# wmeddie/CycloneML

Hardware: AMD Instinct MI355X
Metric: rows/s per training iteration (higher is better)
Workload: dtype f64

## Files before the change

### cycloneml_amd/csrc/kmeans.hip

```cpp
#pragma clang fp contract(off)

#include <hip/hip_runtime.h>

#include <algorithm>
#include <cmath>
#include <cstdlib>
#include <mutex>
#include <utility>
#include <vector>

#include "common.hpp"
#include "kmeans_centers.hpp"
#include "kmeans_i8.hpp"
#include "kmeans_cos.hpp"
#include "kmeans_fp64.hpp"
#include "kmeans_sparse.hpp"
#include "kmeans_sums.hpp"
#include "silhouette.hpp"

namespace {

using cyc::kmsums::kChunkRows;
using cyc::kmsums::kMaxK;

bool env_is0(const char* name) {
  const char* e = std::getenv(name);
  return e && e[0] == '0';
}
int sw_assign_variant() {
  const char* v = std::getenv("CYC_KMEANS_ASSIGN");
  return v ? std::atoi(v) : 0;
}
bool sw_cands3() { return !env_is0("CYC_KMEANS_CANDS3"); }
bool sw_refine() { return std::getenv("CYC_KMEANS_NO_REFINE") == nullptr; }
bool sw_stage() { return std::getenv("CYC_KMEANS_NO_STAGE") == nullptr; }
bool sw_bounds() {
  static const bool on = !env_is0("CYC_KMEANS_BOUNDS");
  return on;
}
bool sw_nbr() {
  static const bool on = !env_is0("CYC_KMEANS_NBR");
  return on;
}
bool sw_incr() {
  static const bool on = !env_is0("CYC_KMEANS_INCR");
  return on;
}
bool sw_exact_split() {
  static const bool on = !env_is0("CYC_KMEANS_EXACT_SPLIT");
  return on;
}
bool sw_list16() {
  static const bool on = !env_is0("CYC_KMEANS_LIST_BM");
  return on;
}
int sw_dump_call() {
  static const int call = [] {
    const char* e = std::getenv("CYC_KMEANS_DUMP_CALL");
    return e ? std::atoi(e) : 10;
  }();
  return call;
}

constexpr int kNormRows = 256, kNormCols = 16, kNormStride = kNormCols + 1;
__global__ __launch_bounds__(kNormRows) void k_row_norms(const double* __restrict__ X, int64_t n,
                                                         int d, double* __restrict__ norms) {
  __shared__ double tile[2][kNormRows * kNormStride];
  const int t = threadIdx.x;
  const int64_t row0 = (int64_t)blockIdx.x * kNormRows;
  constexpr int PER = kNormRows * kNormCols / kNormRows;
  double v[PER];
  auto load = [&](int c0) {
#pragma unroll
    for (int i = 0; i < PER; ++i) {
      const int e = t + kNormRows * i, r = e / kNormCols, c = c0 + e % kNormCols;
      const int64_t gr = row0 + r;
      v[i] = (gr < n && c < d) ? __builtin_nontemporal_load(&X[gr * d + c]) : 0.0;
    }
  };
  auto store = [&](double* b) {
#pragma unroll
    for (int i = 0; i < PER; ++i) {
      const int e = t + kNormRows * i;
      b[(e / kNormCols) * kNormStride + e % kNormCols] = v[i];
    }
  };
// ... 104 lines not shown
    if (c0 + kNormCols < d) store(tile[buf ^ 1]);
    buf ^= 1;
  }
  if (myr < n) cost[myr] = s;
}

}

struct cyc_kmeans_plan_s {
  int d = 0, k = 0;
  int measure = CYC_DISTANCE_EUCLIDEAN;
  cyc::DeviceBuffer cosV, cosVn, cosCn;
  bool dense_ok = true;
  cyc::kmfp64::Sizing fp;
  int64_t lastTier2 = 0;
  int64_t lastExact = 0;
  int64_t lastLimb3 = -1;
  int64_t lastCands = -1;
  int64_t lastCands2 = -1;
  bool cands3 = false;
  cyc::DeviceBuffer cb3, cq3, ok3, list3, list3Count;
  int ktp8 = 0;
  cyc::DeviceBuffer cb8, cq8, g8, prm8, scr8, list8Count;
  cyc::DeviceBuffer candRows, cands, candCount;
  cyc::DeviceBuffer candRows2, cands2, candCount2;
  cyc::DeviceBuffer cand1Rows, cand1, cand1Count, fullList, fullCount;
  cyc::DeviceBuffer stgRowsA, stgRowsB, stgCandRows, stgCands, stgCounts;
  bool lastRefined = false;
  int64_t max_rows = 0;
  std::mutex mu;
  cyc::DeviceBuffer ct, stats, dmin, slowList, slowCount, assignTmp, costTmp;
  cyc::kmsums::SortScratch sort;
  cyc::DeviceBuffer exactDist;
  cyc::DeviceBuffer req;
  cyc::DeviceBuffer silFlags, silNorms, silPart;
  unsigned long long* reqHost = nullptr;
  hipEvent_t reqEv = nullptr;
  ~cyc_kmeans_plan_s() {
    if (reqHost) (void)hipHostFree(reqHost);
    if (reqEv) (void)hipEventDestroy(reqEv);
  }
};

struct cyc_kmeans_rows_s {
  const double* X = nullptr;
  int64_t n = 0;
  int d = 0;
  bool usable = false;
  bool cosine = false;
  cyc::DeviceBuffer img, meta, unorm;
  bool bEnabled = true;
  bool bValid = false;
  int bk = 0;
  cyc::DeviceBuffer bnd, bAssign, bCp, bDelta, bCcs, bPrm, bTmp, bCount, bList, bListCount, bCum;
  cyc::DeviceBuffer bTmp2, bCount2;
  cyc::DeviceBuffer bLnc, bSets, bState, bRc, bRcCount, bRcCum;
  cyc::DeviceBuffer bNbr, bNbrR;
  int64_t bCalls = 0, bFullRows = 0;
  cyc::kmsums::IncState inc;
};

namespace {

int do_stats(cyc_kmeans_plan p, const double* C, hipStream_t st) {
  const int k = p->k, d = p->d;
  const int tps = (k + kStT - 1) / kStT;
// ... 254 lines not shown
                       i8 ? (unsigned int*)p->list3Count.ptr : nullptr);
    CYC_LAUNCH_CHECK("k_zero2");
  }
  int rc = CYC_OK;
  const int32_t* rowList = nullptr;
  const unsigned int* rowCount = nullptr;
  if (i8) {
    if (!a.prepared &&
        (rc = cyc::km8::centers_prepare(C, cnorm, p->k, p->d, p->ktp8, p->cb8.ptr,
                                        (float*)p->cq8.ptr, (double*)p->g8.ptr,
                                        (cyc::km8::CenterParams*)p->prm8.ptr,
                                        (double*)p->scr8.ptr, st)))
      return rc;
    cyc::km8::ScreenCall sc = ss.call;
    sc.xnorm = xnorm;
    sc.assign = a.assign;
    sc.st = st;
    if ((rc = cyc::km8::screen(sc, (int32_t*)p->list3.ptr, (unsigned int*)p->list3Count.ptr,
                               slowList, (unsigned int*)p->list8Count.ptr, ss.cand(),
                               ss.refine(), ss.stage(), a.bounds, a.prepared)))
      return rc;
    rowList = (const int32_t*)p->list3.ptr;
    rowCount = (const unsigned int*)p->list3Count.ptr;
  } else if (fp.variant == 3) {
    if ((rc = cyc::kmfp64::launch_assign3(fp, X, xnorm, n, C, cnorm, p->cb3.ptr,
                                          (float*)p->cq3.ptr, (int*)p->ok3.ptr, a.assign, a.cost,
                                          (int32_t*)p->list3.ptr,
                                          (unsigned int*)p->list3Count.ptr, st)))
      return rc;
    rowList = (const int32_t*)p->list3.ptr;
    rowCount = (const unsigned int*)p->list3Count.ptr;
  }
  const int bm = rowList && sw_list16() && fp.bm >= 16 ? 16 : fp.bm;
  if ((rc = cyc::kmfp64::launch_assign(fp, bm, X, xnorm, n, C, cnorm, ct, a.assign, a.cost,
                                       slowList, slowCount, st, rowList, rowCount)))
    return rc;
  int64_t known = -1;
  if (a.n_exact_out) {
    unsigned int h_slow = 0, h_tier2 = 0, h_limb3 = 0, h_cand = 0, h_cand2 = 0;
    const bool twoPass = i8 && cyc::km8::uses32(p->d);
    CYC_HIP(hipMemcpyAsync(&h_slow, slowCount, sizeof(unsigned), hipMemcpyDeviceToHost, st));
    if (rowCount)
      CYC_HIP(hipMemcpyAsync(&h_tier2, rowCount, sizeof(unsigned), hipMemcpyDeviceToHost, st));
    if (twoPass) {
      CYC_HIP(hipMemcpyAsync(&h_limb3, p->list8Count.ptr, sizeof(unsigned), hipMemcpyDeviceToHost, st));
      CYC_HIP(hipMemcpyAsync(&h_cand, p->candCount.ptr, sizeof(unsigned), hipMemcpyDeviceToHost, st));
      if (p->cands3)
        CYC_HIP(hipMemcpyAsync(&h_cand2, p->candCount2.ptr, sizeof(unsigned), hipMemcpyDeviceToHost, st));
    }
    CYC_HIP(hipStreamSynchronize(st));
    *a.n_exact_out = h_slow;
    p->lastTier2 = rowCount ? (int64_t)h_tier2 : n;
    p->lastExact = h_slow;
    p->lastLimb3 = twoPass ? (int64_t)h_limb3 : -1;
    p->lastCands = twoPass ? (int64_t)h_cand : -1;
    p->lastCands2 = twoPass && p->cands3 ? (int64_t)h_cand2 : -1;
    if (!h_slow) return CYC_OK;
    known = h_slow;
  }
  return cyc::kmfp64::launch_exact(fp, X, xnorm, n, C, cnorm, ct, statsArg, slowList, slowCount,
                                   p->exactDist, a.assign, a.cost, a.approxNorm, known,
                                   sw_exact_split(), st);
}

int req_reserve(cyc_kmeans_plan p, size_t bytes) {
  int rc;
  if ((rc = p->req.reserve(bytes))) return rc;
  if (!p->reqHost) CYC_HIP(hipHostMalloc((void**)&p->reqHost, 5 * sizeof(unsigned long long)));
  if (!p->reqEv) CYC_HIP(hipEventCreateWithFlags(&p->reqEv, hipEventDisableTiming));
  return CYC_OK;
}

int require_enqueue(cyc_kmeans_plan p, const double* C, const double* xnorm, int64_t n,
                    hipStream_t st) {
  int rc;
  if ((rc = req_reserve(p, 5 * sizeof(unsigned long long)))) return rc;
  CYC_HIP(hipMemsetAsync(p->req.ptr, 0xff, 2 * sizeof(unsigned long long), st));
  const int64_t work = std::max<int64_t>(n, (int64_t)p->k * p->d);
  const unsigned grid = (unsigned)std::max<int64_t>(1, std::min<int64_t>((work + 255) / 256, 2048));
  hipLaunchKernelGGL(k_require_norms, dim3(grid), dim3(256), 0, st, C, p->k, p->d, xnorm, n,
                     (unsigned long long*)p->req.ptr);
  CYC_LAUNCH_CHECK("k_require_norms");
  CYC_HIP(hipMemcpyAsync(p->reqHost, p->req.ptr, 5 * sizeof(unsigned long long),
                         hipMemcpyDeviceToHost, st));
  CYC_HIP(hipEventRecord(p->reqEv, st));
  return CYC_OK;
}

int prep_all(cyc_kmeans_plan p, cyc_kmeans_rows rows, const double* xnorm, int64_t n,
             const double* C, const double* cnorm, bool useBnd, bool carry,
             const ScreenSetup* ss, hipStream_t st) {
  namespace k8 = cyc::km8;
  const int k = p->k, d = p->d;
  int rc;
  const size_t reqBytes = sizeof(unsigned long long) * (8 + (size_t)k);
// ... 203 lines not shown
  auto* p = new cyc_kmeans_plan_s();
  p->d = d;
  p->k = k;
  p->fp = cyc::kmfp64::sizing(d, k, sw_assign_variant());
  p->dense_ok = p->fp.bm != 0;
  int rc;
  if (p->fp.variant == 3 &&
      ((rc = p->cb3.reserve((size_t)p->fp.ktp3 * p->fp.ks3 * 2 * 64 * 16)) ||
       (rc = p->cq3.reserve(sizeof(float) * (size_t)p->fp.ktp3 * 16)) ||
       (rc = p->ok3.reserve(64)))) {
    delete p;
    return rc;
  }
  if ((rc = p->list3Count.reserve(64))) {
    delete p;
    return rc;
  }
  if (d <= cyc::km8::kMaxD) {
    const int ks8 = cyc::km8::ksteps(d);
    p->ktp8 = (int)cyc::round_up((k + 15) / 16, cyc::km8::kWaves);
    if ((rc = p->cb8.reserve((size_t)p->ktp8 * ks8 * 3 * 64 * 16 * 2)) ||
        (rc = p->cq8.reserve(sizeof(float) * (size_t)p->ktp8 * 48)) ||
        (rc = p->g8.reserve(sizeof(double) * (size_t)p->ktp8 * 48)) ||
        (rc = p->list8Count.reserve(64)) ||
        (rc = p->prm8.reserve(sizeof(cyc::km8::CenterParams))) ||
        (rc = p->scr8.reserve(sizeof(double) * 2 * (size_t)k))) {
      delete p;
      return rc;
    }
  }
  if ((p->dense_ok && (rc = p->ct.reserve(sizeof(double) * (size_t)p->fp.d4 * p->fp.kpad))) ||
      (rc = p->stats.reserve(sizeof(double) * ((size_t)k * (k + 1) / 2))) ||
      (rc = p->dmin.reserve(sizeof(unsigned long long) * (size_t)k)) ||
      (rc = p->slowCount.reserve(64)) || (rc = ensure_rows(p, std::max<int64_t>(max_rows, 1)))) {
    delete p;
    return rc;
  }
  *plan = p;
  return CYC_OK;
}

int cyc_kmeans_last_tiers(cyc_kmeans_plan p, int64_t* fp64_screen_rows, int64_t* exact_rows) {
  CYC_REQUIRE(p != nullptr && fp64_screen_rows && exact_rows, "arguments must not be null");
  std::lock_guard<std::mutex> g(p->mu);
  *fp64_screen_rows = p->lastTier2;
  *exact_rows = p->lastExact;
  return CYC_OK;
}

int cyc_kmeans_last_screen(cyc_kmeans_plan p, int64_t* three_limb_rows) {
  CYC_REQUIRE(p != nullptr && three_limb_rows, "arguments must not be null");
  std::lock_guard<std::mutex> g(p->mu);
  *three_limb_rows = p->lastLimb3;
  return CYC_OK;
}

int cyc_kmeans_last_candidates(cyc_kmeans_plan p, int64_t* candidate_rows) {
  CYC_REQUIRE(p != nullptr && candidate_rows, "arguments must not be null");
  std::lock_guard<std::mutex> g(p->mu);
  *candidate_rows = p->lastCands;
  return CYC_OK;
}

int cyc_kmeans_last_candidates3(cyc_kmeans_plan p, int64_t* fp64_rows) {
  CYC_REQUIRE(p != nullptr && fp64_rows, "arguments must not be null");
  std::lock_guard<std::mutex> g(p->mu);
  *fp64_rows = p->lastCands2;
// ... 590 lines not shown
```

### cycloneml_amd/csrc/kmeans_fp64.hip

```cpp
#pragma clang fp contract(off)

#include <hip/hip_runtime.h>

#include <algorithm>

#include "common.hpp"
#include "kmeans_fp64.hpp"

namespace {

constexpr int kWaves = 8;
constexpr int kAssignThreads = kWaves * 64;

struct Slot {
  float L1, U1, L2;
  int I1;
};

__device__ __forceinline__ float ulp_down(float f) {
  int b = __float_as_int(f);
  if (f == 0.0f) return -__int_as_float(1);
  return __int_as_float(f > 0.0f ? b - 1 : b + 1);
}
__device__ __forceinline__ float f_down(double x) {
// ... 186 lines not shown
  }
  __syncthreads();

  if (tid < rows) {
    const int row = tid;
    Slot S{__builtin_inff(), __builtin_inff(), __builtin_inff(), -1};
    for (int w = 0; w < kWaves; ++w) {
      const double* m = mrg + ((size_t)w * BM + row) * 4;
      slot_merge(S, (float)m[0], (float)m[1], (float)m[2], (int)m[3]);
    }
    const int64_t grow = CYC_GROW1(row);
    if (S.I1 >= 0 && S.L2 > S.U1) {
      if (cost) {
        const double* crow = C + (int64_t)S.I1 * d;
        const double* xrow = Xs + row * ldsStride;
        double s = 0.0;
        for (int j = 0; j < d; ++j) {
          double sc = dsub(crow[j], xrow[j]);
          s = dadd(s, dmul(sc, sc));
        }
        cost[grow] = s;
      }
      assign[grow] = S.I1;
    } else {
      unsigned slot = atomicAdd(slowCount, 1u);
      slowList[slot] = (int32_t)grow;
    }
  }
  __syncthreads();
  }
#undef CYC_GROW1
}

template <int BM>
__global__ __launch_bounds__(kAssignThreads, 1) void k_kmeans_assign2(
    const double* __restrict__ X, const double* __restrict__ xnorm, int64_t n, int d, int d4,
    int ldsStride, const double* __restrict__ Ct, const double* __restrict__ C,
    const double* __restrict__ cnorm, int k, int kpad, double marginFac,
    int32_t* __restrict__ assign, double* __restrict__ cost, int32_t* __restrict__ slowList,
    unsigned int* __restrict__ slowCount, const int32_t* __restrict__ rowList,
    const unsigned int* __restrict__ rowCount) {
  constexpr int T = BM / 16;
  extern __shared__ __attribute__((aligned(16))) double smem[];
  double* Xs = smem;
  double* xnS = Xs + BM * ldsStride;
  double* mrg = xnS + BM;
  double* cnS = mrg + kWaves * BM * 4;
  double* xqS = cnS + kpad;
  const int64_t nsrc = rowList ? (int64_t)*rowCount : n;
  for (int64_t blk = blockIdx.x; blk * BM < nsrc; blk += gridDim.x) {
#define CYC_GROW(i) (rowList ? (int64_t)rowList[row0 + (i)] : row0 + (i))
  const double fac2 = 2.0 * marginFac;

  const int tid = threadIdx.x, lane = tid & 63;
  const int wave = __builtin_amdgcn_readfirstlane(tid >> 6);
  const int64_t row0 = blk * BM;
  const int rows = (int)min<int64_t>(BM, nsrc - row0);
  {
    const int total = rows * d;
    for (int e = tid; e < total; e += kAssignThreads) {
      int r = e / d, c = e - r * d;
      Xs[r * ldsStride + c] = X[CYC_GROW(r) * d + c];
    }
    for (int e = tid; e < BM * d4; e += kAssignThreads) {
      int r = e / d4, c = e - r * d4;
      if (r >= rows || c >= d) Xs[r * ldsStride + c] = 0.0;
    }
    if (tid < BM) {
      const double xn = (tid < rows) ? xnorm[CYC_GROW(tid)] : 0.0;
      xnS[tid] = xn;
      xqS[tid] = (xn * xn) * (1.0 - fac2);
    }
    for (int c = tid; c < kpad; c += kAssignThreads) cnS[c] = c < k ? cnorm[c] : 0.0;
  }
  __syncthreads();
  const auto ctR = __builtin_amdgcn_make_buffer_rsrc((void*)Ct, (short)0, d4 * kpad * 8,
                                                     0x00020000);
  const int laneOff = ((lane >> 4) * kpad + (lane & 15)) * 8;

  float sL1[T * 4], sL2[T * 4];
  int sI1[T * 4];
#pragma unroll
  for (int q = 0; q < T * 4; ++q) {
    sL1[q] = sL2[q] = __builtin_inff();
    sI1[q] = -1;
  }
  unsigned poison = 0;
  const double* arow = Xs + (lane & 15) * ldsStride + (lane >> 4);
  cyc_double4 acc[T];
  const int G = d4 / 32;
  const int nslabs = (kpad - wave * 16 + kWaves * 16 - 1) / (kWaves * 16);
  const int total = nslabs * G;
  double b0[8], b1[8];

#define CYC_LOADB(B, I)                                                              \
  do {                                                                               \
    const int nb_ = wave * 16 + ((I) / G) * (kWaves * 16);                           \
    const int so_ = ((((I) % G) * 32) * kpad + nb_) * 8;                             \
    _Pragma("unroll") for (int s = 0; s < 8; ++s)                                    \
      B[s] = __builtin_bit_cast(double, __builtin_amdgcn_raw_buffer_load_b64(          \
          ctR, laneOff, so_ + s * 32 * kpad, 0));                                    \
  } while (0)
#define CYC_COMPUTE(B, I)                                                            \
  do {                                                                               \
    const int g_ = (I) % G;                                                          \
    if (g_ == 0) {                                                                   \
      _Pragma("unroll") for (int t = 0; t < T; ++t) acc[t] = cyc_double4{0.0, 0.0, 0.0, 0.0}; \
    }                                                                                \
    _Pragma("unroll") for (int s = 0; s < 8; ++s) {                                  \
      _Pragma("unroll") for (int t = 0; t < T; ++t) {                                \
        const double a_ = arow[t * 16 * ldsStride + g_ * 32 + s * 4];                \
        acc[t] = __builtin_amdgcn_mfma_f64_16x16x4f64(a_, B[s], acc[t], 0, 0, 0);    \
      }                                                                              \
    }                                                                                \
    if (g_ == G - 1) {                                                               \
      const int c_ = wave * 16 + ((I) / G) * (kWaves * 16) + (lane & 15);            \
      const double cn_ = cnS[c_];                                                    \
      const double cq_ = (cn_ * cn_) * (1.0 - fac2);                                 \
      const bool cok_ = c_ < k;                                                      \
      _Pragma("unroll") for (int t = 0; t < T; ++t) {                                \
        _Pragma("unroll") for (int r = 0; r < 4; ++r) {                              \
          const int q = 4 * t + r;                                                   \
          const double xq = xqS[t * 16 + (lane >> 4) + 4 * r];                       \
          const double L = (xq + cq_) - (acc[t][r] + acc[t][r]);                      \
          poison |= (cok_ && !(L == L)) ? (1u << q) : 0u;                            \
          const float fL = (float)L;      \
          const bool lt = cok_ && fL < sL1[q];                                       \
          const float l2 = cok_ ? fminf(sL2[q], fL) : sL2[q];                        \
          sL2[q] = lt ? sL1[q] : l2;                                                 \
          sI1[q] = lt ? c_ : sI1[q];                                                 \
          sL1[q] = lt ? fL : sL1[q];                                                 \
        }                                                                            \
      }                                                                              \
    }                                                                                \
  } while (0)
  __builtin_amdgcn_s_setreg(0x801, 2);
  if (total > 0) CYC_LOADB(b0, 0);
  for (int i = 0; i < total; i += 2) {
    if (i + 1 < total) CYC_LOADB(b1, i + 1);
    CYC_COMPUTE(b0, i);
    if (i + 2 < total) CYC_LOADB(b0, i + 2);
    if (i + 1 < total) CYC_COMPUTE(b1, i + 1);
  }
  __builtin_amdgcn_s_setreg(0x801, 0);
#undef CYC_LOADB
#undef CYC_COMPUTE

#pragma unroll
  for (int q = 0; q < T * 4; ++q) {
#pragma unroll
    for (int m = 1; m < 16; m <<= 1) {
      const float oL1 = __shfl_xor(sL1[q], m), oL2 = __shfl_xor(sL2[q], m);
      const int oI1 = __shfl_xor(sI1[q], m);
      const float hi = fmaxf(sL1[q], oL1);
      sL2[q] = fminf(hi, fminf(sL2[q], oL2));
      const bool take = oL1 < sL1[q] || (oL1 == sL1[q] && oI1 >= 0 && (sI1[q] < 0 || oI1 < sI1[q]));
      sI1[q] = take ? oI1 : sI1[q];
      sL1[q] = take ? oL1 : sL1[q];
    }
  }
#pragma unroll
  for (int m = 1; m < 16; m <<= 1) poison |= __shfl_xor(poison, m);
  if ((lane & 15) == 0) {
#pragma unroll
    for (int t = 0; t < T; ++t) {
#pragma unroll
      for (int r = 0; r < 4; ++r) {
        const int q = 4 * t + r;
        double* m = mrg + ((size_t)wave * BM + t * 16 + (lane >> 4) + 4 * r) * 4;
        m[0] = sL1[q];
        m[1] = ((poison >> q) & 1u) ? -__builtin_inf() : (double)sL2[q];
        m[2] = (double)sI1[q];
      }
    }
  }
  __syncthreads();

  if (tid < rows) {
    const int row = tid;
    float L1 = __builtin_inff(), L2 = __builtin_inff();
    int I1 = -1;
    for (int w = 0; w < kWaves; ++w) {
      const double* m = mrg + ((size_t)w * BM + row) * 4;
      const float oL1 = (float)m[0], oL2 = (float)m[1];
      const int oI1 = (int)m[2];
      const float hi = fmaxf(L1, oL1);
      L2 = fminf(hi, fminf(L2, oL2));
      if (oL1 < L1 || (oL1 == L1 && oI1 >= 0 && (I1 < 0 || oI1 < I1))) {
        L1 = oL1;
        I1 = oI1;
      }
    }
    const int64_t grow = CYC_GROW(row);
    bool decided = false;
    if (I1 >= 0 && L1 == L1 && L1 < __builtin_inff()) {
      const double xn = xnS[row], cn = cnS[I1];
      const double M = (xn * xn + cn * cn) * fac2;
      const double U = (double)(-ulp_down(-L1)) + 2.0 * M * (1.0 + 0x1p-40);
      decided = (double)L2 > U;
    }
    if (decided) {
      if (cost) {
        const double* crow = C + (int64_t)I1 * d;
        const double* xrow = Xs + row * ldsStride;
        double s = 0.0;
        for (int j = 0; j < d; ++j) {
          double sc = dsub(crow[j], xrow[j]);
          s = dadd(s, dmul(sc, sc));
        }
        cost[grow] = s;
      }
      assign[grow] = I1;
    } else {
      unsigned slot = atomicAdd(slowCount, 1u);
      slowList[slot] = (int32_t)grow;
    }
  }
  __syncthreads();
  }
#undef CYC_GROW
}

typedef __bf16 cyc_bf16x8 __attribute__((ext_vector_type(8)));
typedef float cyc_float4 __attribute__((ext_vector_type(4)));

// ... 268 lines not shown
                                                    const int32_t* __restrict__ slowList,
                                                    const unsigned int* __restrict__ slowCount,
                                                    double* __restrict__ dist) {
  __shared__ double xs[1280];
  const unsigned cnt = *slowCount;
  const unsigned idx = blockIdx.y;
  if (cnt > (unsigned)kExactCap || idx >= cnt) return;
  const int tid = threadIdx.x;
  const int c = blockIdx.x * 256 + tid;
  const int64_t r = slowList[idx];
  const double* x = X + r * d;
  const bool xl = d <= 1280;
  if (xl)
    for (int j = tid; j < d; j += 256) xs[j] = x[j];
  __syncthreads();
  const double* xv = xl ? xs : x;
  double acc = 0.0;
  for (int j0 = 0; j0 < d; j0 += 16) {
    double cv[16];
#pragma unroll
    for (int jj = 0; jj < 16; ++jj)
      cv[jj] = (j0 + jj < d && c < k) ? Ct[(int64_t)(j0 + jj) * kpad + c] : 0.0;
#pragma unroll
    for (int jj = 0; jj < 16; ++jj) {
      if (j0 + jj < d) {
        const double sc = dsub(cv[jj], xv[j0 + jj]);
        acc = dadd(acc, dmul(sc, sc));
      }
    }
  }
  if (c < k) dist[(int64_t)idx * kpad + c] = acc;
}

__global__ __launch_bounds__(64) void k_exact_replay(const double* __restrict__ X,
                                                     const double* __restrict__ xnorm, int d,
                                                     int kpad, const double* __restrict__ cnorm,
                                                     int k, const double* __restrict__ stats,
                                                     const int32_t* __restrict__ slowList,
                                                     const unsigned int* __restrict__ slowCount,
                                                     const double* __restrict__ dist,
                                                     int32_t* __restrict__ assign,
                                                     double* __restrict__ cost, int exactNorm) {
  const unsigned cnt = *slowCount;
  const unsigned idx = blockIdx.x;
  if (cnt > (unsigned)kExactCap || idx >= cnt) return;
  const int lane = threadIdx.x;
  const int64_t r = slowList[idx];
  const bool ns = stats == nullptr;
  double xn = 0.0;
  if (exactNorm) {
    if (lane == 0) xn = seq_norm2(X + r * d, d);
    xn = __shfl(xn, 0);
  } else {
    xn = xnorm[r];
  }
  const double* dds = dist + (int64_t)idx * kpad;
  double best = __builtin_inf();
  int bi = 0;
  bool done = false;
  int first = 0;
  if (!ns) {
    best = dds[0];
    done = best < stats[0];
    first = 1;
  }
  for (int i0 = first; !done && i0 < k; i0 += 64) {
    const int i = i0 + lane;
    const bool valid = i < k;
    double lb = __builtin_inf(), sii = 0.0, dd = 0.0;
    if (valid) {
      const double nd = dsub(cnorm[i], xn);
      lb = dmul(nd, nd);
      sii = ns ? 0.0 : stats[iut(i, i)];
      dd = dds[i];
    }
    int pos = 0;
    for (;;) {
      const bool visit = valid && lane >= pos && lb < best && (ns || stats[iut(i, bi)] < best);
      const bool brk = !ns && visit && dd < sii;
      const bool ev = visit && (brk || dd < best);
      const unsigned long long m = __ballot(ev);
      if (!m) break;
      const int f = __ffsll((long long)m) - 1;
      best = __shfl(dd, f);
      bi = i0 + f;
      if (__shfl((int)brk, f)) {
        done = true;
        break;
      }
      pos = f + 1;
    }
  }
  if (lane == 0) {
    assign[r] = bi;
    if (cost) cost[r] = best;
  }
}

constexpr int kExactChunk = 1024;
constexpr int kExactX = 1280;

__global__ __launch_bounds__(256) void k_assign_exact(
    const double* __restrict__ X, const double* __restrict__ xnorm, int d,
    const double* __restrict__ C, const double* __restrict__ Ct, int kpad,
    const double* __restrict__ cnorm, int k,
    const double* __restrict__ stats, const int32_t* __restrict__ slowList,
    const unsigned int* __restrict__ slowCount, int32_t* __restrict__ assign,
    double* __restrict__ cost, int exactNorm, unsigned int skipUpTo) {
  __shared__ double xs[kExactX];
  __shared__ double dds[kExactChunk];
  __shared__ int doneS;
  __shared__ double xnS;
  const unsigned cnt = *slowCount;
  if (cnt <= skipUpTo) return;
  const int tid = threadIdx.x, lane = tid & 63;
  const bool ns = stats == nullptr;
  for (unsigned idx = blockIdx.x; idx < cnt; idx += gridDim.x) {
    const int64_t r = slowList[idx];
    const double* x = X + r * d;
    __syncthreads();
    const bool xl = d <= kExactX;
    if (xl)
      for (int j = tid; j < d; j += 256) xs[j] = x[j];
    const double* xv = xl ? xs : x;
    if (exactNorm) {
      __syncthreads();
      if (tid == 0) xnS = seq_norm2(xv, d);
      __syncthreads();
// ... 74 lines not shown
    }
    if (tid == 0) {
      assign[r] = bi;
      if (cost) cost[r] = best;
    }
  }
}

}

namespace cyc {
namespace kmfp64 {

namespace {

constexpr int kS3TB = 2;

int pick_bm(int d4, int& stride, size_t& lds) {
  const int cands[3] = {64, 32, 16};
  const int maxbm = 64;
  for (int bm : cands) {
    if (bm > maxbm) continue;
    int s = d4 + ((2 - d4 % 32) + 32) % 32;
    size_t bytes = ((size_t)bm * s + bm + (size_t)kWaves * bm * 4) * sizeof(double);
    if (bytes <= 160 * 1024) {
      stride = s;
      lds = bytes;
      return bm;
    }
  }
  return 0;
}

template <int BM>
int launch_assign_bm(const Sizing& s, const double* X, const double* xnorm, int64_t n,
                     const double* C, const double* cnorm, const double* ct, int32_t* assign,
                     double* cost, int32_t* slowList, unsigned int* slowCount, hipStream_t st,
                     const int32_t* rowList, const unsigned int* rowCount) {
  static bool attr_set = false;
  if (!attr_set) {
    CYC_HIP(hipFuncSetAttribute((const void*)k_kmeans_assign<BM>,
                                hipFuncAttributeMaxDynamicSharedMemorySize, 160 * 1024));
    CYC_HIP(hipFuncSetAttribute(reinterpret_cast<const void*>(&k_kmeans_assign2<BM>),
                                hipFuncAttributeMaxDynamicSharedMemorySize, 160 * 1024));
    attr_set = true;
  }
  const double marginFac = (double)(s.d + 16) * 0x1p-46;
  const int64_t blocks = rowList ? std::min<int64_t>((n + BM - 1) / BM, 1024) : (n + BM - 1) / BM;
  cyc::KernelTimer timer(rowList ? "k_kmeans_assign_fp64" : "k_kmeans_assign", st);
  if (s.variant == 2 || s.variant == 3)
    hipLaunchKernelGGL(HIP_KERNEL_NAME(k_kmeans_assign2<BM>), dim3((unsigned)blocks),
                       dim3(kAssignThreads), s.assignLds2, st, X, xnorm, n, s.d, s.d4,
                       s.ldsStride2, ct, C, cnorm, s.k, s.kpad, marginFac, assign, cost, slowList,
                       slowCount, rowList, rowCount);
  else
    hipLaunchKernelGGL(k_kmeans_assign<BM>, dim3((unsigned)blocks), dim3(kAssignThreads),
                       s.assignLds, st, X, xnorm, n, s.d, s.d4, s.ldsStride, ct, C, cnorm, s.k,
                       s.kpad, marginFac, assign, cost, slowList, slowCount, rowList, rowCount);
  CYC_LAUNCH_CHECK("k_kmeans_assign");
  return CYC_OK;
}

}

Sizing sizing(int d, int k, int want) {
  Sizing s;
  s.d = d;
  s.k = k;
  s.d4 = (int)cyc::round_up(d, 4);
  s.kpad = (int)cyc::round_up(k, 16);
  s.bm = pick_bm(s.d4, s.ldsStride, s.assignLds);
  s.ldsStride2 = s.d4 + 1;
  s.assignLds2 = s.assignLds + sizeof(double) * ((size_t)s.kpad + s.bm) -
                 sizeof(double) * (size_t)s.bm * (s.ldsStride - s.ldsStride2);
  s.variant = ((s.d4 % 32) == 0 && s.assignLds2 <= 160 * 1024) ? 2 : 1;
  s.ks3 = (int)((d + 31) / 32);
  s.lds3 = (size_t)2 * kS3BM * (s.ks3 * 4 + 1) * 16 + (size_t)kS3Waves * kS3BM * 12 +
           (size_t)kS3BM * 8;
  const bool fits3 = s.variant == 2 && s.lds3 <= 160 * 1024;
  if (fits3) s.variant = 3;
  if (want == 1 || (s.d4 % 32 == 0 && s.assignLds2 <= 160 * 1024 && want >= 2 && want <= 3 &&
                    (want != 3 || fits3)))
    s.variant = want;
  s.ktp3 = (int)cyc::round_up((k + 15) / 16, kS3Waves * kS3TB);
  const double d32 = 32.0 * s.ks3;
  const double eps = 3.1 * 0x1p-16 + 2.0 * 1.03 * (3.0 * d32 + 64.0) * 0x1p-23 + 0x1p-20;
  const double tau = 0x1p-58;
  s.omE3 = 1.0 - eps;
  s.tauL3 = 2.0 * tau;
  s.facU3 = (2.0 * eps + 0x1p-20) * (1.0 + 0x1p-20);
  s.tauU3 = 4.0 * tau;
  return s;
}

int launch_assign(const Sizing& s, int bm, const double* X, const double* xnorm, int64_t n,
                  const double* C, const double* cnorm, const double* ct, int32_t* assign,
                  double* cost, int32_t* slowList, unsigned int* slowCount, hipStream_t st,
                  const int32_t* rowList, const unsigned int* rowCount) {
  switch (bm) {
    case 64:
      return launch_assign_bm<64>(s, X, xnorm, n, C, cnorm, ct, assign, cost, slowList, slowCount,
                                  st, rowList, rowCount);
    case 32:
      return launch_assign_bm<32>(s, X, xnorm, n, C, cnorm, ct, assign, cost, slowList, slowCount,
                                  st, rowList, rowCount);
    default:
      return launch_assign_bm<16>(s, X, xnorm, n, C, cnorm, ct, assign, cost, slowList, slowCount,
                                  st, rowList, rowCount);
  }
}

int launch_assign3(const Sizing& s, const double* X, const double* xnorm, int64_t n,
                   const double* C, const double* cnorm, void* cb3, float* cq3, int* ok3,
                   int32_t* assign, double* cost, int32_t* list3, unsigned int* list3Count,
                   hipStream_t st) {
  static bool attr_set = false;
  if (!attr_set) {
    CYC_HIP(hipFuncSetAttribute(reinterpret_cast<const void*>(&k_kmeans_assign3<kS3TB>),
                                hipFuncAttributeMaxDynamicSharedMemorySize, 160 * 1024));
    attr_set = true;
  }
  CYC_HIP(hipMemsetAsync(list3Count, 0, sizeof(unsigned int), st));
  CYC_HIP(hipMemsetAsync(ok3, 1, sizeof(int), st));
  const int64_t tot = (int64_t)s.ktp3 * s.ks3 * 64;
  hipLaunchKernelGGL(k_center_split, dim3((unsigned)((tot + 255) / 256)), dim3(256), 0, st, C,
                     cnorm, s.k, s.d, s.ks3, s.ktp3, s.omE3, (uint4*)cb3, cq3, ok3);
  CYC_LAUNCH_CHECK("k_center_split");
  cyc::KernelTimer timer("k_kmeans_assign", st);
  hipLaunchKernelGGL(HIP_KERNEL_NAME(k_kmeans_assign3<kS3TB>),
                     dim3((unsigned)((n + kS3BM - 1) / kS3BM)), dim3(kS3Threads), s.lds3, st, X,
                     xnorm, n, s.d, s.ks3, (const uint4*)cb3, (const float*)cq3, s.ktp3,
                     (const int*)ok3, C, cnorm, s.omE3, s.tauL3, s.facU3, s.tauU3, assign, cost,
                     list3, list3Count);
  CYC_LAUNCH_CHECK("k_kmeans_assign3");
  return CYC_OK;
}

int launch_exact(const Sizing& s, const double* X, const double* xnorm, int64_t n,
                 const double* C, const double* cnorm, const double* ct, const double* statsArg,
                 const int32_t* slowList, const unsigned int* slowCount, DeviceBuffer& exactDist,
                 int32_t* assign, double* cost, bool approxNorm, int64_t known, bool allowSplit,
                 hipStream_t st) {
  cyc::KernelTimer timer("k_kmeans_exact", st);
  const int k = s.k, kpad = s.kpad;
  const bool split = allowSplit && s.d <= 1280 && (known < 0 || known <= kExactCap);
  if (split) {
    int rc;
    if ((rc = exactDist.reserve(sizeof(double) * (size_t)kExactCap * kpad))) return rc;
    const unsigned rowsMax = (unsigned)std::min<int64_t>(known < 0 ? n : known, kExactCap);
    hipLaunchKernelGGL(k_exact_dist, dim3((unsigned)((k + 255) / 256), rowsMax), dim3(256), 0, st,
                       X, s.d, ct, kpad, k, slowList, slowCount, (double*)exactDist.ptr);
    CYC_LAUNCH_CHECK("k_exact_dist");
    hipLaunchKernelGGL(k_exact_replay, dim3(rowsMax), dim3(64), 0, st, X, xnorm, s.d, kpad, cnorm,
                       k, statsArg, slowList, slowCount, (const double*)exactDist.ptr, assign,
                       cost, approxNorm ? 1 : 0);
    CYC_LAUNCH_CHECK("k_exact_replay");
    if (known >= 0) return CYC_OK;
  }
  const unsigned grid = known >= 0 ? (unsigned)std::min<int64_t>(known, 4096)
                                   : (unsigned)std::min<int64_t>((n + 3) / 4, 2048);
  hipLaunchKernelGGL(k_assign_exact, dim3(grid), dim3(256), 0, st, X, xnorm, s.d, C, ct, kpad,
                     cnorm, k, statsArg, slowList, slowCount, assign, cost, approxNorm ? 1 : 0,
                     split ? (unsigned)kExactCap : 0u);
  CYC_LAUNCH_CHECK("k_assign_exact");
  return CYC_OK;
}

}
}
```

### cycloneml_amd/csrc/kmeans_fp64.hpp

```cpp
#pragma once

#include <hip/hip_runtime.h>

#include <cstddef>
#include <cstdint>

#include "common.hpp"

namespace cyc {
namespace kmfp64 {

struct Sizing {
  int d = 0, k = 0, d4 = 0, kpad = 0;
  int bm = 0, ldsStride = 0;
  size_t assignLds = 0;
  int variant = 1;
  int ldsStride2 = 0;
  size_t assignLds2 = 0;
  int ks3 = 0, ktp3 = 0;
  size_t lds3 = 0;
  double omE3 = 1.0, tauL3 = 0.0, facU3 = 0.0, tauU3 = 0.0;
};

Sizing sizing(int d, int k, int want);

int launch_assign(const Sizing& s, int bm, const double* X, const double* xnorm, int64_t n,
                  const double* C, const double* cnorm, const double* ct, int32_t* assign,
                  double* cost, int32_t* slowList, unsigned int* slowCount, hipStream_t st,
                  const int32_t* rowList = nullptr, const unsigned int* rowCount = nullptr);

int launch_assign3(const Sizing& s, const double* X, const double* xnorm, int64_t n,
                   const double* C, const double* cnorm, void* cb3, float* cq3, int* ok3,
                   int32_t* assign, double* cost, int32_t* list3, unsigned int* list3Count,
                   hipStream_t st);

int launch_exact(const Sizing& s, const double* X, const double* xnorm, int64_t n,
                 const double* C, const double* cnorm, const double* ct, const double* statsArg,
                 const int32_t* slowList, const unsigned int* slowCount, DeviceBuffer& exactDist,
                 int32_t* assign, double* cost, bool approxNorm, int64_t known, bool allowSplit,
                 hipStream_t st);

}
}
```

Baseline: 14.21 billion.

## Split short fp64 rescore queues across centroid slabs and fuse exact pass

When the fp64 rescore list is short, the assign2 kernel now splits each row tile's centroid slabs across up to eight blocks. Each block writes partial top-two results, and a ticket-based last-arriver merges them, so more of the GPU is busy on small lists. The exact fallback path fuses distance computation and replay into one k_exact_short kernel using tickets, and the gather of X rows into LDS is batched to expose more loads at once. The cost is extra global partial buffers, atomics and fences, and tighter occupancy bounds that could increase register pressure.

Measured after the change: 14.09 billion. No clear change (-0.9%).

```diff
diff --git a/cycloneml_amd/csrc/kmeans.hip b/cycloneml_amd/csrc/kmeans.hip
--- a/cycloneml_amd/csrc/kmeans.hip
+++ b/cycloneml_amd/csrc/kmeans.hip
@@ -52,6 +52,10 @@
 }
 bool sw_list16() {
   static const bool on = !env_is0("CYC_KMEANS_LIST_BM");
+  return on;
+}
+bool sw_short_queue() {
+  static const bool on = !env_is0("CYC_KMEANS_SHORT_QUEUE");
   return on;
 }
 int sw_dump_call() {
@@ -222,6 +226,8 @@
   cyc::DeviceBuffer ct, stats, dmin, slowList, slowCount, assignTmp, costTmp;
   cyc::kmsums::SortScratch sort;
   cyc::DeviceBuffer exactDist;
+  cyc::DeviceBuffer sqBuf;
+  cyc::kmfp64::ShortQueue sq;
   cyc::DeviceBuffer req;
   cyc::DeviceBuffer silFlags, silNorms, silPart;
   unsigned long long* reqHost = nullptr;
@@ -542,8 +548,9 @@
     rowCount = (const unsigned int*)p->list3Count.ptr;
   }
   const int bm = rowList && sw_list16() && fp.bm >= 16 ? 16 : fp.bm;
+  const cyc::kmfp64::ShortQueue* sq = sw_short_queue() ? &p->sq : nullptr;
   if ((rc = cyc::kmfp64::launch_assign(fp, bm, X, xnorm, n, C, cnorm, ct, a.assign, a.cost,
-                                       slowList, slowCount, st, rowList, rowCount)))
+                                       slowList, slowCount, st, rowList, rowCount, sq)))
     return rc;
   int64_t known = -1;
   if (a.n_exact_out) {
@@ -570,7 +577,7 @@
   }
   return cyc::kmfp64::launch_exact(fp, X, xnorm, n, C, cnorm, ct, statsArg, slowList, slowCount,
                                    p->exactDist, a.assign, a.cost, a.approxNorm, known,
-                                   sw_exact_split(), st);
+                                   sw_exact_split(), st, sq);
 }
 
 int req_reserve(cyc_kmeans_plan p, size_t bytes) {
@@ -840,7 +847,8 @@
   if ((p->dense_ok && (rc = p->ct.reserve(sizeof(double) * (size_t)p->fp.d4 * p->fp.kpad))) ||
       (rc = p->stats.reserve(sizeof(double) * ((size_t)k * (k + 1) / 2))) ||
       (rc = p->dmin.reserve(sizeof(unsigned long long) * (size_t)k)) ||
-      (rc = p->slowCount.reserve(64)) || (rc = ensure_rows(p, std::max<int64_t>(max_rows, 1)))) {
+      (rc = p->slowCount.reserve(64)) ||
+      (rc = cyc::kmfp64::short_queue_reserve(p->sqBuf, p->sq)) || (rc = ensure_rows(p, std::max<int64_t>(max_rows, 1)))) {
     delete p;
     return rc;
   }
diff --git a/cycloneml_amd/csrc/kmeans_fp64.hip b/cycloneml_amd/csrc/kmeans_fp64.hip
--- a/cycloneml_amd/csrc/kmeans_fp64.hip
+++ b/cycloneml_amd/csrc/kmeans_fp64.hip
@@ -242,14 +242,20 @@
 #undef CYC_GROW1
 }
 
-template <int BM>
-__global__ __launch_bounds__(kAssignThreads, 1) void k_kmeans_assign2(
+constexpr int kSqMaxSplit = 8;
+constexpr int kSqMaxGrid = 2048;
+constexpr int kSqTickets = kSqMaxGrid / 2;
+constexpr int kSqPerCu = 2;
+
+template <int BM, bool SQ>
+__global__ __launch_bounds__(kAssignThreads, SQ ? 2 * kSqPerCu : 1) void k_kmeans_assign2(
     const double* __restrict__ X, const double* __restrict__ xnorm, int64_t n, int d, int d4,
     int ldsStride, const double* __restrict__ Ct, const double* __restrict__ C,
     const double* __restrict__ cnorm, int k, int kpad, double marginFac,
     int32_t* __restrict__ assign, double* __restrict__ cost, int32_t* __restrict__ slowList,
     unsigned int* __restrict__ slowCount, const int32_t* __restrict__ rowList,
-    const unsigned int* __restrict__ rowCount) {
+    const unsigned int* __restrict__ rowCount, uint4* __restrict__ sqParts,
+    unsigned int* __restrict__ sqTickets) {
   constexpr int T = BM / 16;
   extern __shared__ __attribute__((aligned(16))) double smem[];
   double* Xs = smem;
@@ -258,7 +264,13 @@
   double* cnS = mrg + kWaves * BM * 4;
   double* xqS = cnS + kpad;
   const int64_t nsrc = rowList ? (int64_t)*rowCount : n;
-  for (int64_t blk = blockIdx.x; blk * BM < nsrc; blk += gridDim.x) {
+  const int64_t tiles = (nsrc + BM - 1) / BM;
+  int S = 1;
+  if constexpr (SQ)
+    while (S < kSqMaxSplit && tiles * (2 * S) <= (int64_t)gridDim.x) S *= 2;
+  for (int64_t item = blockIdx.x; item < tiles * S; item += gridDim.x) {
+  const int64_t blk = item / S;
+  const int split = (int)(item - blk * S);
 #define CYC_GROW(i) (rowList ? (int64_t)rowList[row0 + (i)] : row0 + (i))
   const double fac2 = 2.0 * marginFac;
 
@@ -268,9 +280,30 @@
   const int rows = (int)min<int64_t>(BM, nsrc - row0);
   {
     const int total = rows * d;
-    for (int e = tid; e < total; e += kAssignThreads) {
-      int r = e / d, c = e - r * d;
-      Xs[r * ldsStride + c] = X[CYC_GROW(r) * d + c];
+    if constexpr (SQ) {
+      int64_t* growS = (int64_t*)mrg;
+      if (tid < rows) growS[tid] = CYC_GROW(tid);
+      __syncthreads();
+      for (int e0 = 0; e0 < total; e0 += 8 * kAssignThreads) {
+        double v[8];
+#pragma unroll
+        for (int u = 0; u < 8; ++u) {
+          const int e = e0 + u * kAssignThreads + tid;
+          const int r = e / d, c = e - r * d;
+          v[u] = e < total ? X[growS[r] * d + c] : 0.0;
+        }
+#pragma unroll
+        for (int u = 0; u < 8; ++u) {
+          const int e = e0 + u * kAssignThreads + tid;
+          const int r = e / d, c = e - r * d;
+          if (e < total) Xs[r * ldsStride + c] = v[u];
+        }
+      }
+    } else {
+      for (int e = tid; e < total; e += kAssignThreads) {
+        int r = e / d, c = e - r * d;
+        Xs[r * ldsStride + c] = X[CYC_GROW(r) * d + c];
+      }
     }
     for (int e = tid; e < BM * d4; e += kAssignThreads) {
       int r = e / d4, c = e - r * d4;
@@ -299,13 +332,15 @@
   const double* arow = Xs + (lane & 15) * ldsStride + (lane >> 4);
   cyc_double4 acc[T];
   const int G = d4 / 32;
-  const int nslabs = (kpad - wave * 16 + kWaves * 16 - 1) / (kWaves * 16);
+  const int wslabs = (kpad - wave * 16 + kWaves * 16 - 1) / (kWaves * 16);
+  const int nslabs = wslabs > split ? (wslabs - split + S - 1) / S : 0;
   const int total = nslabs * G;
   double b0[8], b1[8];
 
+#define CYC_SLAB(I) (wave * 16 + (split + ((I) / G) * S) * (kWaves * 16))
 #define CYC_LOADB(B, I)                                                              \
   do {                                                                               \
-    const int nb_ = wave * 16 + ((I) / G) * (kWaves * 16);                           \
+    const int nb_ = CYC_SLAB(I);                                                     \
     const int so_ = ((((I) % G) * 32) * kpad + nb_) * 8;                             \
     _Pragma("unroll") for (int s = 0; s < 8; ++s)                                    \
       B[s] = __builtin_bit_cast(double, __builtin_amdgcn_raw_buffer_load_b64(          \
@@ -324,7 +359,7 @@
       }                                                                              \
     }                                                                                \
     if (g_ == G - 1) {                                                               \
-      const int c_ = wave * 16 + ((I) / G) * (kWaves * 16) + (lane & 15);            \
+      const int c_ = CYC_SLAB(I) + (lane & 15);                                      \
       const double cn_ = cnS[c_];                                                    \
       const double cq_ = (cn_ * cn_) * (1.0 - fac2);                                 \
       const bool cok_ = c_ < k;                                                      \
@@ -355,6 +390,7 @@
   __builtin_amdgcn_s_setreg(0x801, 0);
 #undef CYC_LOADB
 #undef CYC_COMPUTE
+#undef CYC_SLAB
 
 #pragma unroll
   for (int q = 0; q < T * 4; ++q) {
@@ -386,21 +422,60 @@
   }
   __syncthreads();
 
+  float L1 = __builtin_inff(), L2 = __builtin_inff();
+  int I1 = -1;
+#define CYC_MERGE(OL1, OL2, OI1)                                                     \
+  do {                                                                               \
+    const float oL1 = (OL1), oL2 = (OL2);                                            \
+    const int oI1 = (OI1);                                                           \
+    const float hi = fmaxf(L1, oL1);                                                 \
+    L2 = fminf(hi, fminf(L2, oL2));                                                  \
+    if (oL1 < L1 || (oL1 == L1 && oI1 >= 0 && (I1 < 0 || oI1 < I1))) {               \
+      L1 = oL1;                                                                      \
+      I1 = oI1;                                                                      \
+    }                                                                                \
+  } while (0)
   if (tid < rows) {
+    for (int w = 0; w < kWaves; ++w) {
+      const double* m = mrg + ((size_t)w * BM + tid) * 4;
+      CYC_MERGE((float)m[0], (float)m[1], (int)m[2]);
+    }
+  }
+  bool tail = true;
+  if constexpr (SQ) {
+    if (S > 1) {
+      uint4* part = sqParts + (size_t)blk * S * BM;
+      if (tid < rows) {
+        part[split * BM + tid] = uint4{(unsigned)__float_as_int(L1), (unsigned)__float_as_int(L2),
+                                       (unsigned)I1, 0u};
+        __threadfence();
+      }
+      __syncthreads();
+      int* lastS = (int*)mrg;
+      if (tid == 0) {
+        const bool last = atomicAdd(&sqTickets[blk], 1u) == (unsigned)(S - 1);
+        if (last) atomicExch(&sqTickets[blk], 0u);
+        *lastS = last;
+      }
+      __syncthreads();
+      tail = *lastS != 0;
+      if (tail && tid < rows) {
+        __threadfence();
+        L1 = L2 = __builtin_inff();
+        I1 = -1;
+        for (int sp = 0; sp < S; ++sp) {
+          const unsigned* w = (const unsigned*)(part + sp * BM + tid);
+          const unsigned w0 = __hip_atomic_load(w + 0, __ATOMIC_RELAXED, __HIP_MEMORY_SCOPE_AGENT);
+          const unsigned w1 = __hip_atomic_load(w + 1, __ATOMIC_RELAXED, __HIP_MEMORY_SCOPE_AGENT);
+          const unsigned w2 = __hip_atomic_load(w + 2, __ATOMIC_RELAXED, __HIP_MEMORY_SCOPE_AGENT);
+          CYC_MERGE(__int_as_float((int)w0), __int_as_float((int)w1), (int)w2);
+        }
+      }
+    }
+  }
+#undef CYC_MERGE
+  if (tail && tid < rows) {
     const int row = tid;
-    float L1 = __builtin_inff(), L2 = __builtin_inff();
-    int I1 = -1;
-    for (int w = 0; w < kWaves; ++w) {
-      const double* m = mrg + ((size_t)w * BM + row) * 4;
-      const float oL1 = (float)m[0], oL2 = (float)m[1];
-      const int oI1 = (int)m[2];
-      const float hi = fmaxf(L1, oL1);
-      L2 = fminf(hi, fminf(L2, oL2));
-      if (oL1 < L1 || (oL1 == L1 && oI1 >= 0 && (I1 < 0 || oI1 < I1))) {
-        L1 = oL1;
-        I1 = oI1;
-      }
-    }
     const int64_t grow = CYC_GROW(row);
     bool decided = false;
     if (I1 >= 0 && L1 == L1 && L1 < __builtin_inff()) {
@@ -735,6 +810,87 @@
   if (c < k) dist[(int64_t)idx * kpad + c] = acc;
 }
 
+template <bool COH>
+__device__ __forceinline__ void exact_replay_row(
+    const double* __restrict__ X, const double* __restrict__ xnorm, int d,
+    const double* __restrict__ cnorm, int k, const double* __restrict__ stats, int64_t r,
+    const double* dds, int32_t* __restrict__ assign, double* __restrict__ cost, int exactNorm,
+    int lane) {
+  auto dist_at = [&](int i) -> double {
+    if constexpr (COH)
+      return __builtin_bit_cast(
+          double, __hip_atomic_load((const unsigned long long*)(dds + i), __ATOMIC_RELAXED,
+                                    __HIP_MEMORY_SCOPE_AGENT));
+    else
+      return dds[i];
+  };
+  const bool ns = stats == nullptr;
+  double xn = 0.0;
+  if (exactNorm) {
+    if (lane == 0) xn = seq_norm2(X + r * d, d);
+    xn = __shfl(xn, 0);
+  } else {
+    xn = xnorm[r];
+  }
+  double best = __builtin_inf();
+  int bi = 0;
+  bool done = false;
+  int first = 0;
+  if (!ns) {
+    best = dist_at(0);
+    done = best < stats[0];
+    first = 1;
+  }
+  auto operands = [&](int i, double& lb, double& sii, double& dd) {
+    lb = __builtin_inf(), sii = 0.0, dd = 0.0;
+    if (i < k) {
+      const double nd = dsub(cnorm[i], xn);
+      lb = dmul(nd, nd);
+      sii = ns ? 0.0 : stats[iut(i, i)];
+      dd = dist_at(i);
+    }
+  };
+  double nlb = __builtin_inf(), nsii = 0.0, ndd = 0.0, gst = 0.0;
+  int gbi = -1;
+  if (COH && !done && first < k) operands(first + lane, nlb, nsii, ndd);
+  for (int i0 = first; !done && i0 < k; i0 += 64) {
+    const int i = i0 + lane;
+    const bool valid = i < k;
+    double lb, sii, dd;
+    double cst = 0.0;
+    int cbi = -1;
+    if constexpr (COH) {
+      lb = nlb, sii = nsii, dd = ndd, cst = gst, cbi = gbi;
+      operands(i + 64, nlb, nsii, ndd);
+      gst = (!ns && i + 64 < k) ? stats[iut(i + 64, bi)] : 0.0;
+      gbi = bi;
+    } else {
+      operands(i, lb, sii, dd);
+    }
+    int pos = 0;
+    for (;;) {
+      const bool visit = valid && lane >= pos && lb < best &&
+                         (ns || (bi == cbi ? cst : stats[iut(i, bi)]) < best);
+      const bool brk = !ns && visit && dd < sii;
+      const bool ev = visit && (brk || dd < best);
+      const unsigned long long m = __ballot(ev);
+      if (!m) break;
+      const int f = __ffsll((long long)m) - 1;
+      best = __shfl(dd, f);
+      bi = i0 + f;
+      if (__shfl((int)brk, f)) {
+        done = true;
+        break;
+      }
+      pos = f + 1;
+    }
+  }
+  if (lane == 0) {
+    assign[r] = bi;
+    if (cost) cost[r] = best;
+  }
+}
+
 __global__ __launch_bounds__(64) void k_exact_replay(const double* __restrict__ X,
                                                      const double* __restrict__ xnorm, int d,
                                                      int kpad, const double* __restrict__ cnorm,
@@ -747,56 +903,70 @@
   const unsigned cnt = *slowCount;
   const unsigned idx = blockIdx.x;
   if (cnt > (unsigned)kExactCap || idx >= cnt) return;
-  const int lane = threadIdx.x;
-  const int64_t r = slowList[idx];
-  const bool ns = stats == nullptr;
-  double xn = 0.0;
-  if (exactNorm) {
-    if (lane == 0) xn = seq_norm2(X + r * d, d);
-    xn = __shfl(xn, 0);
-  } else {
-    xn = xnorm[r];
-  }
-  const double* dds = dist + (int64_t)idx * kpad;
-  double best = __builtin_inf();
-  int bi = 0;
-  bool done = false;
-  int first = 0;
-  if (!ns) {
-    best = dds[0];
-    done = best < stats[0];
-    first = 1;
-  }
-  for (int i0 = first; !done && i0 < k; i0 += 64) {
-    const int i = i0 + lane;
-    const bool valid = i < k;
-    double lb = __builtin_inf(), sii = 0.0, dd = 0.0;
-    if (valid) {
-      const double nd = dsub(cnorm[i], xn);
-      lb = dmul(nd, nd);
-      sii = ns ? 0.0 : stats[iut(i, i)];
-      dd = dds[i];
-    }
-    int pos = 0;
-    for (;;) {
-      const bool visit = valid && lane >= pos && lb < best && (ns || stats[iut(i, bi)] < best);
-      const bool brk = !ns && visit && dd < sii;
-      const bool ev = visit && (brk || dd < best);
-      const unsigned long long m = __ballot(ev);
-      if (!m) break;
-      const int f = __ffsll((long long)m) - 1;
-      best = __shfl(dd, f);
-      bi = i0 + f;
-      if (__shfl((int)brk, f)) {
-        done = true;
-        break;
-      }
-      pos = f + 1;
-    }
-  }
-  if (lane == 0) {
-    assign[r] = bi;
-    if (cost) cost[r] = best;
+  exact_replay_row<false>(X, xnorm, d, cnorm, k, stats, slowList[idx], dist + (int64_t)idx * kpad,
+                          assign, cost, exactNorm, threadIdx.x);
+}
+
+constexpr int kExactBlk = 64;
+
+__global__ __launch_bounds__(256) void k_exact_short(
+    const double* __restrict__ X, const double* __restrict__ xnorm, int d,
+    const double* __restrict__ Ct, int kpad, const double* __restrict__ cnorm, int k,
+    const double* __restrict__ stats, const int32_t* __restrict__ slowList,
+    const unsigned int* __restrict__ slowCount, double* __restrict__ dist,
+    unsigned int* __restrict__ tickets, int32_t* __restrict__ assign, double* __restrict__ cost,
+    int exactNorm) {
+  __shared__ double xs[1280];
+  __shared__ int lastS;
+  const unsigned cnt = *slowCount;
+  if (cnt > (unsigned)kExactCap) return;
+  const int tid = threadIdx.x;
+  const int c = blockIdx.x * 256 + tid;
+  const bool cok = c < k;
+  const double* col = Ct + (cok ? c : 0);
+  for (unsigned idx = blockIdx.y; idx < cnt; idx += gridDim.y) {
+    const int64_t r = slowList[idx];
+    const double* x = X + r * d;
+    __syncthreads();
+    for (int j = tid; j < d; j += 256) xs[j] = x[j];
+    __syncthreads();
+    double acc = 0.0;
+    double cva[kExactBlk], cvb[kExactBlk];
+#define CYC_XLOAD(CV, J0)                                                            \
+  _Pragma("unroll") for (int jj = 0; jj < kExactBlk; ++jj)                           \
+      CV[jj] = col[(int64_t)min((J0) + jj, d - 1) * kpad]
+#define CYC_XADD(CV, J0)                                                             \
+  _Pragma("unroll") for (int jj = 0; jj < kExactBlk; ++jj) {                         \
+    if ((J0) + jj < d) {                                                             \
+      const double sc = dsub(CV[jj], xs[(J0) + jj]);                                 \
+      acc = dadd(acc, dmul(sc, sc));                                                 \
+    }                                                                                \
+  }
+    CYC_XLOAD(cva, 0);
+    for (int j0 = 0; j0 < d; j0 += 2 * kExactBlk) {
+      if (j0 + kExactBlk < d) CYC_XLOAD(cvb, j0 + kExactBlk);
+      CYC_XADD(cva, j0)
+      if (j0 + 2 * kExactBlk < d) CYC_XLOAD(cva, j0 + 2 * kExactBlk);
+      if (j0 + kExactBlk < d) CYC_XADD(cvb, j0 + kExactBlk)
+    }
+#undef CYC_XLOAD
+#undef CYC_XADD
+    if (cok) {
+      dist[(int64_t)idx * kpad + c] = acc;
+      __threadfence();
+    }
+    __syncthreads();
+    if (tid == 0) {
+      const bool last = atomicAdd(&tickets[idx], 1u) == gridDim.x - 1;
+      if (last) atomicExch(&tickets[idx], 0u);
+      lastS = last;
+    }
+    __syncthreads();
+    if (lastS && tid < 64) {
+      __threadfence();
+      exact_replay_row<true>(X, xnorm, d, cnorm, k, stats, r, dist + (int64_t)idx * kpad, assign,
+                             cost, exactNorm, tid);
+    }
   }
 }
 
@@ -937,27 +1107,59 @@
   return 0;
 }
 
+size_t assign_lds(const Sizing& s, int bm, bool v2) {
+  if (v2)
+    return sizeof(double) * ((size_t)bm * s.ldsStride2 + bm + (size_t)kWaves * bm * 4 + s.kpad + bm);
+  return sizeof(double) * ((size_t)bm * s.ldsStride + bm + (size_t)kWaves * bm * 4);
+}
+
 template <int BM>
 int launch_assign_bm(const Sizing& s, const double* X, const double* xnorm, int64_t n,
                      const double* C, const double* cnorm, const double* ct, int32_t* assign,
                      double* cost, int32_t* slowList, unsigned int* slowCount, hipStream_t st,
-                     const int32_t* rowList, const unsigned int* rowCount) {
+                     const int32_t* rowList, const unsigned int* rowCount, const ShortQueue* sq) {
   static bool attr_set = false;
   if (!attr_set) {
     CYC_HIP(hipFuncSetAttribute((const void*)k_kmeans_assign<BM>,
                                 hipFuncAttributeMaxDynamicSharedMemorySize, 160 * 1024));
-    CYC_HIP(hipFuncSetAttribute(reinterpret_cast<const void*>(&k_kmeans_assign2<BM>),
+    CYC_HIP(hipFuncSetAttribute(reinterpret_cast<const void*>(&k_kmeans_assign2<BM, false>),
                                 hipFuncAttributeMaxDynamicSharedMemorySize, 160 * 1024));
+    if constexpr (BM == 16)
+      CYC_HIP(hipFuncSetAttribute(reinterpret_cast<const void*>(&k_kmeans_assign2<BM, true>),
+                                  hipFuncAttributeMaxDynamicSharedMemorySize, 160 * 1024));
     attr_set = true;
   }
   const double marginFac = (double)(s.d + 16) * 0x1p-46;
+  const bool v2 = s.variant == 2 || s.variant == 3;
+  cyc::KernelTimer timer(rowList ? "k_kmeans_assign_fp64" : "k_kmeans_assign", st);
+  if constexpr (BM == 16) {
+    if (rowList && sq) {
+      const size_t lds = assign_lds(s, BM, v2);
+      int dev = 0, cus = 0;
+      CYC_HIP(hipGetDevice(&dev));
+      CYC_HIP(hipDeviceGetAttribute(&cus, hipDeviceAttributeMultiprocessorCount, dev));
+      const int perCu = v2 ? (int)std::max<size_t>(1, std::min<size_t>(kSqPerCu, 160 * 1024 / lds)) : 1;
+      const int64_t resident = std::min<int64_t>((int64_t)cus * perCu, kSqMaxGrid);
+      const unsigned blocks = (unsigned)std::min<int64_t>((n + BM - 1) / BM, resident);
+      if (v2)
+        hipLaunchKernelGGL(HIP_KERNEL_NAME(k_kmeans_assign2<BM, true>), dim3(blocks),
+                           dim3(kAssignThreads), lds, st, X, xnorm, n, s.d, s.d4, s.ldsStride2, ct,
+                           C, cnorm, s.k, s.kpad, marginFac, assign, cost, slowList, slowCount,
+                           rowList, rowCount, (uint4*)sq->parts, sq->tickets);
+      else
+        hipLaunchKernelGGL(k_kmeans_assign<BM>, dim3(blocks), dim3(kAssignThreads), lds, st, X,
+                           xnorm, n, s.d, s.d4, s.ldsStride, ct, C, cnorm, s.k, s.kpad, marginFac,
+                           assign, cost, slowList, slowCount, rowList, rowCount);
+      CYC_LAUNCH_CHECK("k_kmeans_assign");
+      return CYC_OK;
+    }
+  }
   const int64_t blocks = rowList ? std::min<int64_t>((n + BM - 1) / BM, 1024) : (n + BM - 1) / BM;
-  cyc::KernelTimer timer(rowList ? "k_kmeans_assign_fp64" : "k_kmeans_assign", st);
-  if (s.variant == 2 || s.variant == 3)
-    hipLaunchKernelGGL(HIP_KERNEL_NAME(k_kmeans_assign2<BM>), dim3((unsigned)blocks),
+  if (v2)
+    hipLaunchKernelGGL(HIP_KERNEL_NAME(k_kmeans_assign2<BM, false>), dim3((unsigned)blocks),
                        dim3(kAssignThreads), s.assignLds2, st, X, xnorm, n, s.d, s.d4,
                        s.ldsStride2, ct, C, cnorm, s.k, s.kpad, marginFac, assign, cost, slowList,
-                       slowCount, rowList, rowCount);
+                       slowCount, rowList, rowCount, (uint4*)nullptr, (unsigned int*)nullptr);
   else
     hipLaunchKernelGGL(k_kmeans_assign<BM>, dim3((unsigned)blocks), dim3(kAssignThreads),
                        s.assignLds, st, X, xnorm, n, s.d, s.d4, s.ldsStride, ct, C, cnorm, s.k,
@@ -1001,18 +1203,31 @@
 int launch_assign(const Sizing& s, int bm, const double* X, const double* xnorm, int64_t n,
                   const double* C, const double* cnorm, const double* ct, int32_t* assign,
                   double* cost, int32_t* slowList, unsigned int* slowCount, hipStream_t st,
-                  const int32_t* rowList, const unsigned int* rowCount) {
+                  const int32_t* rowList, const unsigned int* rowCount, const ShortQueue* sq) {
   switch (bm) {
     case 64:
       return launch_assign_bm<64>(s, X, xnorm, n, C, cnorm, ct, assign, cost, slowList, slowCount,
-                                  st, rowList, rowCount);
+                                  st, rowList, rowCount, sq);
     case 32:
       return launch_assign_bm<32>(s, X, xnorm, n, C, cnorm, ct, assign, cost, slowList, slowCount,
-                                  st, rowList, rowCount);
+                                  st, rowList, rowCount, sq);
     default:
       return launch_assign_bm<16>(s, X, xnorm, n, C, cnorm, ct, assign, cost, slowList, slowCount,
-                                  st, rowList, rowCount);
-  }
+                                  st, rowList, rowCount, sq);
+  }
+}
+
+int short_queue_reserve(DeviceBuffer& buf, ShortQueue& sq) {
+  const size_t parts = sizeof(uint4) * (size_t)kSqMaxGrid * 16;
+  const size_t tickets = sizeof(unsigned int) * (size_t)(kSqTickets + kExactCap);
+  int rc;
+  if ((rc = buf.reserve(parts + tickets))) return rc;
+  CYC_HIP(hipMemset((char*)buf.ptr + parts, 0, tickets));
+  CYC_HIP(hipDeviceSynchronize());
+  sq.parts = buf.ptr;
+  sq.tickets = (unsigned int*)((char*)buf.ptr + parts);
+  sq.exactTickets = sq.tickets + kSqTickets;
+  return CYC_OK;
 }
 
 int launch_assign3(const Sizing& s, const double* X, const double* xnorm, int64_t n,
@@ -1045,7 +1260,7 @@
                  const double* C, const double* cnorm, const double* ct, const double* statsArg,
                  const int32_t* slowList, const unsigned int* slowCount, DeviceBuffer& exactDist,
                  int32_t* assign, double* cost, bool approxNorm, int64_t known, bool allowSplit,
-                 hipStream_t st) {
+                 hipStream_t st, const ShortQueue* sq) {
   cyc::KernelTimer timer("k_kmeans_exact", st);
   const int k = s.k, kpad = s.kpad;
   const bool split = allowSplit && s.d <= 1280 && (known < 0 || known <= kExactCap);
@@ -1053,6 +1268,14 @@
     int rc;
     if ((rc = exactDist.reserve(sizeof(double) * (size_t)kExactCap * kpad))) return rc;
     const unsigned rowsMax = (unsigned)std::min<int64_t>(known < 0 ? n : known, kExactCap);
+    if (sq) {
+      const unsigned gx = (unsigned)((k + 255) / 256);
+      const unsigned gy = std::min(rowsMax, std::max(1u, 512u / gx));
+      hipLaunchKernelGGL(k_exact_short, dim3(gx, gy), dim3(256), 0, st, X, xnorm, s.d, ct, kpad,
+                         cnorm, k, statsArg, slowList, slowCount, (double*)exactDist.ptr,
+                         sq->exactTickets, assign, cost, approxNorm ? 1 : 0);
+      CYC_LAUNCH_CHECK("k_exact_short");
+    } else {
     hipLaunchKernelGGL(k_exact_dist, dim3((unsigned)((k + 255) / 256), rowsMax), dim3(256), 0, st,
                        X, s.d, ct, kpad, k, slowList, slowCount, (double*)exactDist.ptr);
     CYC_LAUNCH_CHECK("k_exact_dist");
@@ -1060,6 +1283,7 @@
                        k, statsArg, slowList, slowCount, (const double*)exactDist.ptr, assign,
                        cost, approxNorm ? 1 : 0);
     CYC_LAUNCH_CHECK("k_exact_replay");
+    }
     if (known >= 0) return CYC_OK;
   }
   const unsigned grid = known >= 0 ? (unsigned)std::min<int64_t>(known, 4096)
diff --git a/cycloneml_amd/csrc/kmeans_fp64.hpp b/cycloneml_amd/csrc/kmeans_fp64.hpp
--- a/cycloneml_amd/csrc/kmeans_fp64.hpp
+++ b/cycloneml_amd/csrc/kmeans_fp64.hpp
@@ -24,10 +24,18 @@
 
 Sizing sizing(int d, int k, int want);
 
+struct ShortQueue {
+  void* parts = nullptr;
+  unsigned int* tickets = nullptr;
+  unsigned int* exactTickets = nullptr;
+};
+int short_queue_reserve(DeviceBuffer& buf, ShortQueue& sq);
+
 int launch_assign(const Sizing& s, int bm, const double* X, const double* xnorm, int64_t n,
                   const double* C, const double* cnorm, const double* ct, int32_t* assign,
                   double* cost, int32_t* slowList, unsigned int* slowCount, hipStream_t st,
-                  const int32_t* rowList = nullptr, const unsigned int* rowCount = nullptr);
+                  const int32_t* rowList = nullptr, const unsigned int* rowCount = nullptr,
+                  const ShortQueue* sq = nullptr);
 
 int launch_assign3(const Sizing& s, const double* X, const double* xnorm, int64_t n,
                    const double* C, const double* cnorm, void* cb3, float* cq3, int* ok3,
@@ -38,7 +46,7 @@
                  const double* C, const double* cnorm, const double* ct, const double* statsArg,
                  const int32_t* slowList, const unsigned int* slowCount, DeviceBuffer& exactDist,
                  int32_t* assign, double* cost, bool approxNorm, int64_t known, bool allowSplit,
-                 hipStream_t st);
+                 hipStream_t st, const ShortQueue* sq = nullptr);
 
 }
 }
```
